# arkworks-rs/circom-compat

Measured on NVIDIA H100. Metric: groth16_proofs_per_sec_bn254_2p20, higher is better.
Workload: dtype u32x8 (254-bit Montgomery integers)

## Files before the change

### circom_compat_b200/csrc/msm.cu

```cuda
#include <algorithm>
#include <type_traits>
#include <vector>
#include "msm.cuh"
#include "util.cuh"

namespace b2g {

std::atomic<uint64_t> g_launch_count{0};

template <class C, class F>
__global__ void __launch_bounds__(128) msm_table_kernel(const void* __restrict__ bases, uint32_t n, int c, int nwin, void* __restrict__ table) {
    uint32_t i = blockIdx.x * blockDim.x + threadIdx.x;
    if (i >= n) return;
    using Pt = typename C::Pt; using Aff = typename C::Aff; using E = typename F::elem;
    Aff p = aff_load<F>(bases, i);
    if (C::aff_is_inf(p)) {
        Aff z; z.x = F::zero(); z.y = F::zero();
        for (int w = 0; w < nwin; w++) aff_store<F>(table, (size_t)w * n + i, z);
        return;
    }
    Pt pts[MSM_MAX_WIN];
    E pre[MSM_MAX_WIN];
    Pt cur = C::from_affine(p);
    E acc = F::one();
// ... 150 lines not shown
        const int leader = __ffs(pend) - 1;
        const uint32_t lb = __shfl_sync(0xffffffffu, b, leader);
        const bool mine = pending && b == lb;
        const uint32_t same = __ballot_sync(0xffffffffu, mine);
        uint32_t base = 0;
        if ((int)lane == leader) base = atomicAdd(&cursor[lb], (uint32_t)__popc(same));
        base = __shfl_sync(0xffffffffu, base, leader);
        if (mine) {
            entries[offsets[b] + base + (uint32_t)__popc(same & ((1u << lane) - 1u))] = entry;
            pending = false;
        }
    }
    if (pending) entries[offsets[b] + atomicAdd(&cursor[b], 1u)] = entry;
}

__global__ void __launch_bounds__(1024) msm_aff_levels_kernel(uint32_t nb, int rounds, uint32_t* const* __restrict__ off) {
    __shared__ uint32_t warp_sums[32];
    __shared__ uint32_t carry_s;
    const uint32_t tid = threadIdx.x, per = (nb + 1023u) / 1024u;
    const uint32_t lo = min(tid * per, nb), hi = min(lo + per, nb);
    for (int k = 1; k <= rounds; k++) {
        const uint32_t* prev = off[k - 1];
        uint32_t* cur = off[k];
        uint32_t s = 0;
        for (uint32_t j = lo; j < hi; j++) s += (prev[j + 1] - prev[j] + 1u) >> 1;
        uint32_t v = s;
        #pragma unroll
        for (int d = 1; d < 32; d <<= 1) { uint32_t t = __shfl_up_sync(0xffffffffu, v, d); if ((tid & 31) >= (uint32_t)d) v += t; }
        if ((tid & 31) == 31) warp_sums[tid >> 5] = v;
        __syncthreads();
        if (tid < 32) {
            uint32_t w = warp_sums[tid], x = w;
            #pragma unroll
            for (int d = 1; d < 32; d <<= 1) { uint32_t t = __shfl_up_sync(0xffffffffu, x, d); if (tid >= (uint32_t)d) x += t; }
            warp_sums[tid] = x - w;
            if (tid == 31) carry_s = x;
        }
        __syncthreads();
        uint32_t run = warp_sums[tid >> 5] + v - s;
        for (uint32_t j = lo; j < hi; j++) { cur[j] = run; run += (prev[j + 1] - prev[j] + 1u) >> 1; }
        if (tid == 0) cur[nb] = carry_s;
        __syncthreads();
    }
}

__global__ void __launch_bounds__(256) msm_aff_src_kernel(const uint32_t* __restrict__ off_prev, const uint32_t* __restrict__ off_cur, uint32_t nb,
                                                          uint32_t* __restrict__ src) {
    const uint32_t total = off_cur[nb];
    for (uint32_t q = blockIdx.x * blockDim.x + threadIdx.x; q < total; q += gridDim.x * blockDim.x) {
        uint32_t lo = 0, hi = nb;
        while (hi - lo > 1) { const uint32_t mid = (lo + hi) >> 1; if (off_cur[mid] <= q) lo = mid; else hi = mid; }
        const uint32_t j = q - off_cur[lo];
        const uint32_t p0 = off_prev[lo], cnt = off_prev[lo + 1] - p0;
        src[q] = (p0 + 2u * j) | ((2u * j + 1u < cnt) ? 0x80000000u : 0u);
    }
}

enum : int { AFF_COPY_P = 0, AFF_COPY_Q = 1, AFF_INF = 2, AFF_ADD = 3, AFF_DBL = 4 };

template <class C, class F, bool LEVEL0>
__device__ __forceinline__ int aff_fetch(const void* __restrict__ table, const uint32_t* __restrict__ entries, const void* __restrict__ prev,
                                         uint32_t s, typename C::Aff& P, typename C::Aff& Q, typename F::elem& d) {
    const uint32_t i0 = s & 0x7fffffffu;
    const bool pair = (s >> 31) != 0;
    if (LEVEL0) {
        const uint32_t e0 = entries[i0];
        P = aff_load<F>(table, (size_t)(e0 & 0x7fffffffu));
        if (e0 >> 31) P.y = F::neg(P.y);
        if (pair) {
            const uint32_t e1 = entries[i0 + 1];
            Q = aff_load<F>(table, (size_t)(e1 & 0x7fffffffu));
            if (e1 >> 31) Q.y = F::neg(Q.y);
        }
    } else {
        P = aff_load<F>(prev, (size_t)i0);
        if (pair) Q = aff_load<F>(prev, (size_t)i0 + 1);
    }
    if (!pair) return AFF_COPY_P;
    if (C::aff_is_inf(P)) return AFF_COPY_Q;
    if (C::aff_is_inf(Q)) return AFF_COPY_P;
    if (F::eq(P.x, Q.x)) {
        if (F::eq(P.y, Q.y) && !F::is_zero(P.y)) { d = F::dbl(P.y); return AFF_DBL; }
        return AFF_INF;
    }
    d = F::sub(Q.x, P.x);
    return AFF_ADD;
}

template <class C, class F, bool LEVEL0>
__global__ void __launch_bounds__(128) msm_aff_prod_kernel(const void* __restrict__ table, const uint32_t* __restrict__ entries, const void* __restrict__ prev,
                                                           const uint32_t* __restrict__ src, const uint32_t* __restrict__ off_cur, uint32_t nb,
                                                           void* __restrict__ pref, void* __restrict__ totals) {
    using E = typename F::elem; using Aff = typename C::Aff;
    const uint32_t total = off_cur[nb];
    const uint32_t t = blockIdx.x * blockDim.x + threadIdx.x, stride = gridDim.x * blockDim.x;
    E run = F::one();
    #pragma unroll 1
    for (int i = 0; i < MSM_AFF_M; i++) {
        const uint64_t q64 = (uint64_t)t + (uint64_t)i * stride;
        if (q64 >= total) break;
        const uint32_t q = (uint32_t)q64;
        Aff P, Q; E d;
        const int kind = aff_fetch<C, F, LEVEL0>(table, entries, prev, src[q], P, Q, d);
        if (kind >= AFF_ADD) {
            elem_store((char*)pref + (size_t)q * Bytes<F>::ELEM, run);
            run = F::mul(run, d);
        }
    }
    elem_store((char*)totals + (size_t)t * Bytes<F>::ELEM, run);
}

template <class F>
__global__ void __launch_bounds__(64) msm_aff_invert_kernel(void* __restrict__ totals, void* __restrict__ scratch, uint32_t count, uint32_t U) {
    using E = typename F::elem;
    const uint32_t u = blockIdx.x * blockDim.x + threadIdx.x;
    if (u >= U) return;
    constexpr size_t B = Bytes<F>::ELEM;
    E run = F::one();
    int last = -1;
    #pragma unroll 1
    for (int v = 0; v < MSM_AFF_S; v++) {
        const uint64_t idx = (uint64_t)u + (uint64_t)v * U;
        if (idx >= count) break;
        E x; elem_load(x, (const char*)totals + idx * B);
        elem_store((char*)scratch + idx * B, run);
        run = F::mul(run, x);
        last = v;
    }
    if (last < 0) return;
    E inv = F::inv(run);
    #pragma unroll 1
    for (int v = last; v >= 0; v--) {
        const uint64_t idx = (uint64_t)u + (uint64_t)v * U;
        E x, pre; elem_load(x, (const char*)totals + idx * B); elem_load(pre, (const char*)scratch + idx * B);
        elem_store((char*)totals + idx * B, F::mul(inv, pre));
        inv = F::mul(inv, x);
    }
}

template <class C, class F, bool LEVEL0>
__global__ void __launch_bounds__(128) msm_aff_apply_kernel(const void* __restrict__ table, const uint32_t* __restrict__ entries, const void* __restrict__ prev,
                                                            const uint32_t* __restrict__ src, const uint32_t* __restrict__ off_cur, uint32_t nb,
                                                            const void* __restrict__ pref, const void* __restrict__ totals_inv, void* __restrict__ out) {
    using E = typename F::elem; using Aff = typename C::Aff;
    const uint32_t total = off_cur[nb];
    const uint32_t t = blockIdx.x * blockDim.x + threadIdx.x, stride = gridDim.x * blockDim.x;
    if (t >= total) return;
    E inv; elem_load(inv, (const char*)totals_inv + (size_t)t * Bytes<F>::ELEM);
    int i = MSM_AFF_M - 1;
    while ((uint64_t)t + (uint64_t)i * stride >= total) i--;
    #pragma unroll 1
    for (; i >= 0; i--) {
        const uint32_t q = t + (uint32_t)i * stride;
        Aff P, Q; E d;
        const int kind = aff_fetch<C, F, LEVEL0>(table, entries, prev, src[q], P, Q, d);
        Aff r;
        if (kind >= AFF_ADD) {
            E pre; elem_load(pre, (const char*)pref + (size_t)q * Bytes<F>::ELEM);
            const E inv_d = F::mul(inv, pre);
            inv = F::mul(inv, d);
            E num;
            if (kind == AFF_ADD) num = F::sub(Q.y, P.y);
            else { const E xx = F::sqr(P.x); num = F::add(F::dbl(xx), xx); Q.x = P.x; }
            const E lam = F::mul(num, inv_d);
            r.x = F::sub(F::sub(F::sqr(lam), P.x), Q.x);
            r.y = F::sub(F::mul(lam, F::sub(P.x, r.x)), P.y);
        } else if (kind == AFF_COPY_P) r = P;
        else if (kind == AFF_COPY_Q) r = Q;
        else { r.x = F::zero(); r.y = F::zero(); }
        aff_store<F>(out, (size_t)q, r);
    }
}

template <class F> struct AccOcc;
#ifndef B2G_G1_CTAS
#define B2G_G1_CTAS 4
#endif
template <> struct AccOcc<Fq> { static constexpr int MIN_CTAS = B2G_G1_CTAS; };

__device__ __forceinline__ void acc_stage_slab(uint32_t* slab, unsigned long long* slab_bar, const uint32_t* __restrict__ entries,
                                               uint64_t cta_first, uint32_t total, uint32_t slab_words) {
// ... 246 lines not shown
    CUDA_CHECK(cudaMemsetAsync(flag.d, 0, 4, st));
    if (g2) msm_validate_kernel<G2, Fq2><<<(n + 255) / 256, 256, 0, st>>>(pts_dev, n, flag.d);
    else msm_validate_kernel<G1, Fq><<<(n + 255) / 256, 256, 0, st>>>(pts_dev, n, flag.d);
    g_launch_count += 1;
    CUDA_CHECK(cudaMemcpyAsync(&bad, flag.d, 4, cudaMemcpyDeviceToHost, st));
    CUDA_CHECK(cudaStreamSynchronize(st));
    if (bad) throw_error(B2G_E_INPUT, std::string(g2 ? "G2" : "G1") + " point " + std::to_string(bad - 1) + " of " + what + " is not on the curve");
}

template <class C, class F>
static void msm_build_table_t(MsmPlan& plan, const void* bases_dev, uint32_t n, cudaStream_t st) {
    const size_t aff = 2 * Bytes<F>::ELEM;
    uint32_t c = env_u32("B2G_MSM_C", (uint32_t)msm_pick_c(n ? n : 1));
    if (c < 8 || c > 22) throw_error(B2G_E_SHAPE, "B2G_MSM_C must be in [8, 22]");
    plan.n = n; plan.c = (int)c; plan.nwin = msm_nwin(plan.c); plan.nbuckets = 1u << (plan.c - 1);
    if (n == 0) { plan.table = nullptr; return; }
    if ((uint64_t)n * plan.nwin >= (1ull << 31)) throw_error(B2G_E_SHAPE, "msm: n * windows exceeds 2^31 table rows");
    msm_validate_points(bases_dev, n, plan.g2, st, "the query slice");
    CUDA_CHECK(cudaMalloc(&plan.table, (size_t)n * plan.nwin * aff));
    msm_table_kernel<C, F><<<(n + 127) / 128, 128, 0, st>>>(bases_dev, n, plan.c, plan.nwin, plan.table);
    g_launch_count += 1;
    CUDA_CHECK(cudaGetLastError());
}

void msm_build_table(MsmPlan& plan, const void* bases_dev, uint32_t n, bool g2, cudaStream_t st) {
    plan.g2 = g2;
    if (g2) msm_build_table_t<G2, Fq2>(plan, bases_dev, n, st);
    else msm_build_table_t<G1, Fq>(plan, bases_dev, n, st);
}

void msm_free_table(MsmPlan& plan) { if (plan.table) cudaFree(plan.table); plan.table = nullptr; }

void msm_scratch_alloc(MsmScratch& s, uint32_t n, int nwin, uint32_t nbuckets_one, bool g2, bool with_sort, uint32_t count) {
    s.g2 = g2; s.cap_n = n; s.cap_nwin = nwin; s.cap_buckets = nbuckets_one; s.cap_count = count;
    s.chunk = env_u32(g2 ? "B2G_MSM_CHUNK_G2" : "B2G_MSM_CHUNK", env_u32("B2G_MSM_CHUNK", 64));
    const size_t pt = (g2 ? 4 * 64 : 4 * 32);
    const size_t nent = (size_t)n * nwin * count;
    const size_t nbuckets = (size_t)nbuckets_one * count;
    const size_t nchunks = (nent + s.chunk - 1) / s.chunk + 1;
    s.reduce_chunk = env_u32("B2G_MSM_REDUCE_CHUNK", MSM_REDUCE_CHUNK_DEFAULT);
    {
        const char* bulk_env = getenv("B2G_ACC_BULK");
        s.bulk = bulk_env && *bulk_env ? *bulk_env == '1' : !g2;
    }
    const size_t npart = ((size_t)nbuckets_one / (s.reduce_chunk * 32) + 64) * count;
    if (with_sort) {
        CUDA_CHECK(cudaMalloc(&s.counts, (size_t)nbuckets * 4));
        CUDA_CHECK(cudaMalloc(&s.offsets, ((size_t)nbuckets + 1) * 4));
        CUDA_CHECK(cudaMalloc(&s.cursor, (size_t)nbuckets * 4));
        CUDA_CHECK(cudaMalloc(&s.entries, (nent + 8) * 4));
        CUDA_CHECK(cudaMalloc(&s.scalars_canon, ((size_t)n * count + 1) * sizeof(fe)));
    }
    CUDA_CHECK(cudaMalloc(&s.big_list, (size_t)nbuckets * 4));
    CUDA_CHECK(cudaMalloc(&s.big_count, 4));
    CUDA_CHECK(cudaMalloc(&s.frag_first, nchunks * pt));
    CUDA_CHECK(cudaMalloc(&s.frag_last, nchunks * pt));
    CUDA_CHECK(cudaMalloc(&s.buckets, (size_t)nbuckets * pt));
    CUDA_CHECK(cudaMalloc(&s.partials, (npart + 1) * pt));
    CUDA_CHECK(cudaMalloc(&s.result, pt)); s.result_owned = true;
    {
        int rounds = 0;
        const char* ov = getenv("B2G_MSM_AFFINE_ROUNDS");
        if (ov && *ov) { long x = strtol(ov, nullptr, 10); rounds = x < 0 ? 0 : (x > MSM_AFF_MAX_ROUNDS ? MSM_AFF_MAX_ROUNDS : (int)x); }
        s.aff_cap_rounds = rounds;
        s.aff_nmax[0] = (uint32_t)nent;
        for (int k = 1; k <= rounds; k++) s.aff_nmax[k] = s.aff_nmax[k - 1] / 2 + (uint32_t)(nbuckets / 2) + 1;
        if (rounds) {
            const size_t elem = g2 ? 64 : 32, aff = 2 * elem;
            if (with_sort) {
                std::vector<uint32_t*> offs(MSM_AFF_MAX_ROUNDS + 1, nullptr);
                offs[0] = s.offsets;
                for (int k = 1; k <= rounds; k++) {
                    CUDA_CHECK(cudaMalloc(&s.aff_off[k], ((size_t)nbuckets + 1) * 4));
                    CUDA_CHECK(cudaMalloc(&s.aff_src[k], ((size_t)s.aff_nmax[k] + 1) * 4));
                    offs[k] = s.aff_off[k];
                }
                s.aff_off[0] = s.offsets;
                CUDA_CHECK(cudaMalloc(&s.aff_off_dev, (MSM_AFF_MAX_ROUNDS + 1) * sizeof(uint32_t*)));
                CUDA_CHECK(cudaMemcpy(s.aff_off_dev, offs.data(), (MSM_AFF_MAX_ROUNDS + 1) * sizeof(uint32_t*), cudaMemcpyHostToDevice));
            }
            CUDA_CHECK(cudaMalloc(&s.aff_list[0], ((size_t)s.aff_nmax[1] + 1) * aff));
            if (rounds > 1) CUDA_CHECK(cudaMalloc(&s.aff_list[1], ((size_t)s.aff_nmax[2] + 1) * aff));
            const size_t threads1 = ((size_t)s.aff_nmax[1] + MSM_AFF_M - 1) / MSM_AFF_M + 128;
            CUDA_CHECK(cudaMalloc(&s.aff_pref, ((size_t)s.aff_nmax[1] + 1) * elem));
            CUDA_CHECK(cudaMalloc(&s.aff_totals, threads1 * elem));
            CUDA_CHECK(cudaMalloc(&s.aff_tscratch, threads1 * elem));
        }
    }
    if (env_u32("B2G_MSM_TAIL_PRIORITY", 1) == 1) {
        int least = 0, greatest = 0;
        CUDA_CHECK(cudaDeviceGetStreamPriorityRange(&least, &greatest));
        CUDA_CHECK(cudaStreamCreateWithPriority(&s.tail, cudaStreamNonBlocking, greatest));
        CUDA_CHECK(cudaEventCreateWithFlags(&s.ev_acc, cudaEventDisableTiming));
        CUDA_CHECK(cudaEventCreateWithFlags(&s.ev_tail, cudaEventDisableTiming));
    }
}

void msm_scratch_free(MsmScratch& s) {
    void* ptrs[] = {s.counts, s.offsets, s.cursor, s.entries, s.big_list, s.big_count, s.frag_first, s.frag_last,
                    s.buckets, s.partials, s.result_owned ? s.result : nullptr, s.scalars_canon,
                    s.aff_list[0], s.aff_list[1], s.aff_pref, s.aff_totals, s.aff_tscratch, s.aff_off_dev};
    for (void* p : ptrs) if (p) cudaFree(p);
    for (int k = 1; k <= MSM_AFF_MAX_ROUNDS; k++) { if (s.aff_off[k]) cudaFree(s.aff_off[k]); if (s.aff_src[k]) cudaFree(s.aff_src[k]); }
    if (s.tail) { cudaStreamDestroy(s.tail); cudaEventDestroy(s.ev_acc); cudaEventDestroy(s.ev_tail); }
    s = MsmScratch();
}

void msm_sort(const MsmPlan& plan, MsmScratch& s, const fe* scalars_dev, uint32_t n, bool scalars_mont, cudaStream_t st, uint32_t count,
              uint32_t scalar_stride) {
    if (n > plan.n) n = plan.n;
    s.sorted_n = n; s.sorted_count = count;
    if (n == 0 || plan.table == nullptr) return;
    if (n > s.cap_n || plan.nwin > s.cap_nwin || plan.nbuckets > s.cap_buckets || count > s.cap_count || !s.entries) throw_error(B2G_E_SHAPE, "msm: sort scratch too small");
    const uint32_t nb = plan.nbuckets * count;
    constexpr unsigned SORT_CTA = 256;
    CUDA_CHECK(cudaMemsetAsync(s.counts, 0, (size_t)nb * 4, st));
    const dim3 pair_grid((unsigned)(((uint64_t)n * plan.nwin + SORT_CTA - 1) / SORT_CTA), count);
    msm_canon_kernel<<<dim3((n + SORT_CTA - 1) / SORT_CTA, count), SORT_CTA, 0, st>>>(scalars_dev, n, scalar_stride ? scalar_stride : n, scalars_mont ? 1 : 0, s.scalars_canon);
    msm_count_kernel<<<pair_grid, SORT_CTA, 0, st>>>(s.scalars_canon, n, plan.c, plan.nwin, plan.nbuckets, s.counts);
    msm_scan_kernel<<<1, 1024, 0, st>>>(s.counts, nb, s.offsets, s.cursor);
    msm_scatter_kernel<<<pair_grid, SORT_CTA, 0, st>>>(s.scalars_canon, n, plan.n, plan.c, plan.nwin, plan.nbuckets, s.offsets, s.cursor, s.entries);
    g_launch_count += 4;
    s.aff_rounds = s.aff_off_dev ? s.aff_cap_rounds : 0;
    if (s.aff_rounds) {
        msm_aff_levels_kernel<<<1, 1024, 0, st>>>(nb, s.aff_rounds, s.aff_off_dev);
        for (int k = 1; k <= s.aff_rounds; k++) {
            const unsigned blocks = (unsigned)std::min<uint64_t>(((uint64_t)s.aff_nmax[k] + 255) / 256, 1u << 20);
            msm_aff_src_kernel<<<blocks, 256, 0, st>>>(s.aff_off[k - 1], s.aff_off[k], nb, s.aff_src[k]);
        }
        g_launch_count += 1 + s.aff_rounds;
    }
    CUDA_CHECK(cudaGetLastError());
}

template <class C, class F>
static void launch_accumulate(const void* table, const uint32_t* entries, const uint32_t* offsets, uint32_t nb, uint32_t chunk, uint32_t nruns,
                              const MsmScratch& s, bool bulk, cudaStream_t st) {
    constexpr bool g2 = std::is_same<F, Fq2>::value;
    constexpr uint32_t runs_per_cta = g2 ? 64u : 128u;
    const uint32_t slab_words = bulk && (size_t)chunk * runs_per_cta * 4 <= MSM_SLAB_MAX_BYTES ? chunk * runs_per_cta : 0u;
    const unsigned blocks = (unsigned)(((uint64_t)nruns + runs_per_cta - 1) / runs_per_cta);
    if constexpr (g2)
        msm_accumulate_g2_kernel<<<blocks, 128, (size_t)slab_words * 4, st>>>(table, entries, offsets, nb, chunk, s.buckets, s.frag_first, s.frag_last, slab_words);
    else
        msm_accumulate_kernel<C, F><<<blocks, 128, (size_t)slab_words * 4, st>>>(table, entries, offsets, nb, chunk, s.buckets, s.frag_first, s.frag_last, slab_words);
}

template <class C, class F>
static void msm_accumulate_t(const MsmPlan& plan, const MsmScratch& sorted, MsmScratch& s, cudaStream_t st) {
    using Pt = typename C::Pt;
    const size_t ptb = sizeof(Pt);
    const uint32_t n = sorted.sorted_n, count = sorted.sorted_count;
    const size_t rstride = s.result_stride ? s.result_stride : ptb;
    if (n == 0 || plan.table == nullptr) { CUDA_CHECK(cudaMemset2DAsync(s.result, rstride, 0, ptb, count, st)); return; }
    if (plan.nbuckets > s.cap_buckets || n > s.cap_n || plan.nwin > s.cap_nwin || count > s.cap_count) throw_error(B2G_E_SHAPE, "msm: accumulate scratch too small");
    const uint32_t nb = plan.nbuckets * count, chunk = s.chunk;
    CUDA_CHECK(cudaMemsetAsync(s.big_count, 0, 4, st));
    const uint64_t nent = (uint64_t)n * plan.nwin * count;
    const uint32_t nthreads = (uint32_t)((nent + chunk - 1) / chunk);
    if (s.prof0) CUDA_CHECK(cudaEventRecord(s.prof0, st));
    int rounds = sorted.aff_rounds < s.aff_cap_rounds ? sorted.aff_rounds : s.aff_cap_rounds;
    if (rounds && (sorted.aff_nmax[1] > s.aff_nmax[1] || !s.aff_list[0])) rounds = 0;
    const uint32_t* offsets = sorted.offsets;
    if (rounds) {
        const void* prev = nullptr;
        for (int k = 1; k <= rounds; k++) {
            const uint32_t nk = sorted.aff_nmax[k];
            const unsigned blocks = (unsigned)(((uint64_t)nk + (uint64_t)MSM_AFF_M * 128 - 1) / ((uint64_t)MSM_AFF_M * 128));
            const uint32_t stride = blocks * 128u, U = (stride + MSM_AFF_S - 1) / MSM_AFF_S;
            void* out = s.aff_list[(k - 1) & 1];
            if (k == 1) {
                msm_aff_prod_kernel<C, F, true><<<blocks, 128, 0, st>>>(plan.table, sorted.entries, nullptr, sorted.aff_src[k], sorted.aff_off[k], nb, s.aff_pref, s.aff_totals);
                msm_aff_invert_kernel<F><<<(U + 63) / 64, 64, 0, st>>>(s.aff_totals, s.aff_tscratch, stride, U);
                msm_aff_apply_kernel<C, F, true><<<blocks, 128, 0, st>>>(plan.table, sorted.entries, nullptr, sorted.aff_src[k], sorted.aff_off[k], nb, s.aff_pref, s.aff_totals, out);
            } else {
                msm_aff_prod_kernel<C, F, false><<<blocks, 128, 0, st>>>(nullptr, nullptr, prev, sorted.aff_src[k], sorted.aff_off[k], nb, s.aff_pref, s.aff_totals);
                msm_aff_invert_kernel<F><<<(U + 63) / 64, 64, 0, st>>>(s.aff_totals, s.aff_tscratch, stride, U);
// ... 20 lines not shown
    const uint32_t npart = (nred + NT - 1) / NT;
    msm_reduce_kernel<C, F><<<dim3(npart, count), NT, sh, st>>>(s.buckets, nb1, rchunk, s.partials);
    msm_sum_kernel<C, F><<<count, NT, sh, st>>>(s.partials, npart, s.result, rstride);
    if (s.tail) { CUDA_CHECK(cudaEventRecord(s.ev_tail, s.tail)); CUDA_CHECK(cudaStreamWaitEvent(main_st, s.ev_tail, 0)); }
    g_launch_count += 5;
    CUDA_CHECK(cudaGetLastError());
}

void msm_accumulate(const MsmPlan& plan, const MsmScratch& sorted, MsmScratch& acc, cudaStream_t st) {
    if (plan.g2) msm_accumulate_t<G2, Fq2>(plan, sorted, acc, st);
    else msm_accumulate_t<G1, Fq>(plan, sorted, acc, st);
}

void msm_run(const MsmPlan& plan, MsmScratch& s, const fe* scalars_dev, uint32_t n, bool scalars_mont, cudaStream_t st, uint32_t count,
             uint32_t scalar_stride) {
    msm_sort(plan, s, scalars_dev, n, scalars_mont, st, count, scalar_stride);
    msm_accumulate(plan, s, s, st);
}

void msm_init_kernels() {
    CUDA_CHECK(cudaFuncSetAttribute(msm_accumulate_kernel<G1, Fq>, cudaFuncAttributeMaxDynamicSharedMemorySize, MSM_SLAB_MAX_BYTES));
    CUDA_CHECK(cudaFuncSetAttribute(msm_accumulate_g2_kernel, cudaFuncAttributeMaxDynamicSharedMemorySize, MSM_SLAB_MAX_BYTES));
}

}
```

### circom_compat_b200/csrc/msm.cuh

```cuda
#pragma once
#include "ec.cuh"

namespace b2g {

constexpr int MSM_MAX_WIN = 32;
constexpr int MSM_BIG_FRAGS = 32;

struct MsmPlan {
    uint32_t n = 0;
    int c = 0, nwin = 0;
    uint32_t nbuckets = 0;
    void* table = nullptr;
    bool g2 = false;
};

constexpr int MSM_AFF_MAX_ROUNDS = 6;
constexpr int MSM_AFF_M = 16;
constexpr int MSM_AFF_S = 64;

struct MsmScratch {
    uint32_t cap_n = 0; int cap_nwin = 0; uint32_t cap_buckets = 0; uint32_t chunk = 64; uint32_t sorted_n = 0; uint32_t reduce_chunk = 8;
    uint32_t cap_count = 1, sorted_count = 1;
    size_t result_stride = 0;
    uint32_t *counts = nullptr, *offsets = nullptr, *cursor = nullptr, *entries = nullptr;
    uint32_t *big_list = nullptr, *big_count = nullptr;
    void *frag_first = nullptr, *frag_last = nullptr, *buckets = nullptr, *partials = nullptr, *result = nullptr;
    fe* scalars_canon = nullptr;
    bool g2 = false, result_owned = false;
    bool bulk = false;
    cudaEvent_t prof0 = nullptr, prof1 = nullptr;
    cudaStream_t tail = nullptr;
    cudaEvent_t ev_acc = nullptr, ev_tail = nullptr;
    int aff_rounds = 0;
    int aff_cap_rounds = 0;
    uint32_t aff_nmax[MSM_AFF_MAX_ROUNDS + 1] = {};
    uint32_t* aff_off[MSM_AFF_MAX_ROUNDS + 1] = {};
    uint32_t** aff_off_dev = nullptr;
    uint32_t* aff_src[MSM_AFF_MAX_ROUNDS + 1] = {};
    void* aff_list[2] = {nullptr, nullptr};
    void *aff_pref = nullptr, *aff_totals = nullptr, *aff_tscratch = nullptr;
};

inline int msm_pick_c(uint32_t n) {
    if (n >= 3u << 18) return 17;
    if (n >= 1u << 19) return 16;
    if (n >= 1u << 15) return 15;
    if (n >= 1u << 13) return 13;
    if (n >= 1u << 11) return 11;
    int lg = 0; while ((1ull << (lg + 1)) <= n) lg++;
    return lg - 3 < 8 ? 8 : lg - 3;
}
inline int msm_nwin(int c) { return (255 + c - 1) / c; }

}
```

### circom_compat_b200/csrc/prover.cu

```cuda
#include <atomic>
#include <chrono>
#include <cstring>
#include <vector>
#include "../../include/b2groth.h"
#include "ec.cuh"
#include "msm.cuh"
#include "ntt.cuh"
#include "util.cuh"

namespace b2g {

void msm_build_table(MsmPlan& plan, const void* bases_dev, uint32_t n, bool g2, cudaStream_t st);
void msm_free_table(MsmPlan& plan);
void msm_scratch_alloc(MsmScratch& s, uint32_t n, int nwin, uint32_t nbuckets, bool g2, bool with_sort, uint32_t count = 1);
void msm_sort(const MsmPlan& plan, MsmScratch& s, const fe* scalars_dev, uint32_t n, bool scalars_mont, cudaStream_t st, uint32_t count = 1,
              uint32_t scalar_stride = 0);
void msm_accumulate(const MsmPlan& plan, const MsmScratch& sorted, MsmScratch& acc, cudaStream_t st);
void msm_scratch_free(MsmScratch& s);
void msm_run(const MsmPlan& plan, MsmScratch& s, const fe* scalars_dev, uint32_t n, bool scalars_mont, cudaStream_t st, uint32_t count = 1,
             uint32_t scalar_stride = 0);
void msm_init_kernels();
void msm_validate_points(const void* pts_dev, uint32_t n, bool g2, cudaStream_t st, const char* what);

enum { Q_H = 0, Q_L = 1, Q_A = 2, Q_B1 = 3, Q_B2 = 4, NQ = 5 };
static const size_t PARTIAL_OFF[NQ] = {0, 128, 256, 384, 512};
constexpr size_t REC_BYTES = B2G_PARTIAL_BYTES + 256;
constexpr uint32_t MAX_BATCH = 65535;

}

using namespace b2g;
// ... 512 lines not shown
    ctx->cap_batch = 0; ctx->alloc_gen++;
    if (ctx->scratch_ok) for (int q = 0; q < NQ; q++) ctx->scratch[q].result = nullptr;
    CUDA_CHECK(cudaMalloc(&ctx->d_partial, count * REC_BYTES));
    CUDA_CHECK(cudaMemset(ctx->d_partial, 0, count * REC_BYTES));
    CUDA_CHECK(cudaMalloc(&ctx->d_proof, count * 256));
    CUDA_CHECK(cudaMalloc(&ctx->d_pre, count * PRE_BYTES));
    CUDA_CHECK(cudaMalloc(&ctx->d_rs, count * 64));
    CUDA_CHECK(cudaMallocHost(&ctx->h_rs, count * 64));
    CUDA_CHECK(cudaMallocHost(&ctx->h_proof, count * 256));
    ctx->cap_batch = count;
    if (ctx->scratch_ok) for (int q = 0; q < NQ; q++) ctx->scratch[q].result = ctx->d_partial + PARTIAL_OFF[q];
}

static void ensure_scratch(b2g_ctx* ctx, const b2g_pk* pk, uint32_t count = 1) {
    const size_t nwb = (size_t)pk->b_compact * count;
    bool ok = ctx->scratch_ok && (!pk->d_bidx || (ctx->scratch_bsort && nwb <= ctx->cap_wb));
    for (int q = 0; q < NQ && ok; q++) {
        const MsmPlan& p = pk->plan[q]; const MsmScratch& sc = ctx->scratch[q];
        if ((p.n ? p.n : 1) > sc.cap_n || p.nwin > sc.cap_nwin || p.nbuckets > sc.cap_buckets || count > sc.cap_count) ok = false;
    }
    if (ok) return;
    CUDA_CHECK(cudaDeviceSynchronize());
    for (int q = 0; q < NQ; q++) msm_scratch_free(ctx->scratch[q]);
    ctx->scratch_ok = false; ctx->alloc_gen++;
    for (int q = 0; q < NQ; q++) {
        const MsmPlan& p = pk->plan[q];
        msm_scratch_alloc(ctx->scratch[q], p.n ? p.n : 1, p.nwin, p.nbuckets, q == Q_B2, q == Q_H || q == Q_L || (q == Q_B1 && pk->d_bidx), count);
        cudaFree(ctx->scratch[q].result);
        ctx->scratch[q].result = ctx->d_partial + PARTIAL_OFF[q];
        ctx->scratch[q].result_owned = false;
        ctx->scratch[q].result_stride = REC_BYTES;
    }
    ctx->scratch_bsort = pk->d_bidx != nullptr;
    const size_t nwb_cap = (size_t)pk->b_compact * count;
    if (nwb_cap > ctx->cap_wb) {
        if (ctx->d_wb) cudaFree(ctx->d_wb);
        ctx->d_wb = nullptr; ctx->cap_wb = 0;
        CUDA_CHECK(cudaMalloc(&ctx->d_wb, (nwb_cap + 1) * sizeof(fe)));
        ctx->cap_wb = nwb_cap;
    }
    ctx->scratch_ok = true;
}
// ... 55 lines not shown
        ntt_transform_single(mat->dom, eval, st);
        eval_publish_kernel<<<1, 32, 0, st>>>(ctx->d_xchg, ctx->d_epoch);
        g_launch_count += 1;
    }
    if (cnt) {
        h_slice_kernel<<<(cnt + 255) / 256, 256, 0, st>>>(ctx->d_peer_ptrs, ctx->d_epoch, lo, cnt, ctx->d_h, p2p_timeout_ns(), d_flag);
        g_launch_count += 1;
    }
    CUDA_CHECK(cudaGetLastError());
}

static void launch_msms(b2g_ctx* ctx, b2g_pk* pk, b2g_mat* mat, bool timed, bool scale, bool split_map = false, uint32_t count = 1) {
    cudaStream_t s0 = ctx->st[0], ssort = ctx->st[Q_L];
    CUDA_CHECK(cudaEventRecord(ctx->ev_w, s0));
    CUDA_CHECK(cudaStreamWaitEvent(ssort, ctx->ev_w, 0));
    msm_sort(pk->plan[Q_A], ctx->scratch[Q_L], ctx->d_w + pk->scalar_off[Q_A] + pk->lo[Q_A], pk->cnt[Q_A], true, ssort, count, pk->n_vars);
    CUDA_CHECK(cudaEventRecord(ctx->ev_sort, ssort));
    const bool bsparse = pk->d_bidx != nullptr;
    if (bsparse) {
        cudaStream_t sb = ctx->st[Q_B1];
        CUDA_CHECK(cudaStreamWaitEvent(sb, ctx->ev_w, 0));
        if (pk->b_compact) gather_scalars_kernel<<<dim3((pk->b_compact + 255) / 256, count), 256, 0, sb>>>(ctx->d_w + pk->scalar_off[Q_B1] + pk->lo[Q_B1], pk->n_vars, pk->d_bidx, pk->b_compact, ctx->d_wb);
        g_launch_count += 1;
        msm_sort(pk->plan[Q_B1], ctx->scratch[Q_B1], ctx->d_wb, pk->b_compact, true, sb, count, pk->b_compact);
        CUDA_CHECK(cudaEventRecord(ctx->ev_sortb, sb));
    }
    const int* order = witness_order();
    for (int oi = 0; oi < 4; oi++) {
        const int q = order[oi];
        const bool on_b = bsparse && (q == Q_B1 || q == Q_B2);
        if (on_b) { if (q != Q_B1) CUDA_CHECK(cudaStreamWaitEvent(ctx->st[q], ctx->ev_sortb, 0)); }
        else if (q != Q_L) CUDA_CHECK(cudaStreamWaitEvent(ctx->st[q], ctx->ev_sort, 0));
        if (timed) CUDA_CHECK(cudaEventRecord(ctx->ev_t[2 * q], ctx->st[q]));
        msm_accumulate(pk->plan[q], on_b ? ctx->scratch[Q_B1] : ctx->scratch[Q_L], ctx->scratch[q], ctx->st[q]);
        if (scale && (q == Q_A || q == Q_B1)) {
            const Scalar256* rs = reinterpret_cast<const Scalar256*>(ctx->d_rs);
            scale_partial_kernel<<<count, 32, 0, ctx->st[q]>>>(ctx->d_partial + PARTIAL_OFF[q], q == Q_A ? rs + 1 : rs, ctx->d_partial + B2G_PARTIAL_BYTES + (q == Q_A ? 0 : 128));
            g_launch_count += 1;
        }
        if (timed) CUDA_CHECK(cudaEventRecord(ctx->ev_t[2 * q + 1], ctx->st[q]));
        CUDA_CHECK(cudaEventRecord(ctx->ev_done[q], ctx->st[q]));
    }
    if (timed) CUDA_CHECK(cudaEventRecord(ctx->ev_t[10], s0));
    if (split_map) run_witness_map_split(ctx, mat, pk->lo[Q_H], pk->cnt[Q_H], s0);
    else run_witness_map(ctx, mat, s0, count);
    if (timed) CUDA_CHECK(cudaEventRecord(ctx->ev_t[11], s0));
    if (timed) CUDA_CHECK(cudaEventRecord(ctx->ev_t[0], s0));
    msm_run(pk->plan[Q_H], ctx->scratch[Q_H], ctx->d_h + pk->lo[Q_H], pk->cnt[Q_H], true, s0, count, mat->n);
// ... 689 lines not shown
}

}
template <bool IS_G2>
static void msm_entry(b2g_ctx* ctx, const void* bases, const void* scalars, size_t n, int scalars_mont, void* out) {
    if (!ctx || !out || (n && (!bases || !scalars))) throw_error(B2G_E_SHAPE, "null pointer");
    if (n >= (1ull << 27)) throw_error(B2G_E_SHAPE, "msm too large");
    DevGuard g(ctx->device);
    cudaStream_t st = ctx->st[0];
    const size_t aff = IS_G2 ? 128 : 64, ptb = 2 * aff;
    if (n == 0) { memset(out, 0, aff); return; }
    uint8_t* d_bases = dev_upload<uint8_t>(bases, n * aff, st);
    fe* d_sc = dev_upload<fe>(scalars, n * 32, st);
    MsmPlan plan; MsmScratch sc;
    msm_build_table(plan, d_bases, (uint32_t)n, IS_G2, st);
    msm_scratch_alloc(sc, (uint32_t)n, plan.nwin, plan.nbuckets, IS_G2, true);
    msm_run(plan, sc, d_sc, (uint32_t)n, scalars_mont != 0, st);
    uint8_t* d_out = nullptr; CUDA_CHECK(cudaMalloc(&d_out, aff));
    if (IS_G2) xyzz_to_affine_kernel<G2, Fq2><<<1, 1, 0, st>>>(sc.result, 1, d_out);
    else xyzz_to_affine_kernel<G1, Fq><<<1, 1, 0, st>>>(sc.result, 1, d_out);
    g_launch_count += 2;
    CUDA_CHECK(cudaMemcpyAsync(out, d_out, aff, cudaMemcpyDeviceToHost, st));
    cudaError_t e = cudaStreamSynchronize(st);
    (void)ptb;
    cudaFree(d_out); cudaFree(d_bases); cudaFree(d_sc); msm_free_table(plan); msm_scratch_free(sc);
    CUDA_CHECK(e);
}

extern "C" {
int b2g_msm_g1(b2g_ctx* ctx, const void* bases, const void* scalars, size_t n, int scalars_mont, void* out) {
    return guarded([&] { msm_entry<false>(ctx, bases, scalars, n, scalars_mont, out); });
// ... 80 lines not shown
```

Baseline: 35.94.

## Enable affine batch-inversion bucket rounds for large G2 MSMs by default

Turns on two rounds of affine pairwise bucket reduction with Montgomery batch inversion for G2 MSMs of size 2^18 or more. Before, this path was only reachable through an environment variable. The level-offset kernel now computes each round's offsets in parallel from the base offsets, one block per round, instead of looping serially. The product kernel prefetches sort entries and loads only x coordinates to form denominators, and Fq2 uses inline mul/sqr. When a single consumer needs levels, their planning moves onto that consumer's stream, at the cost of extra scratch memory and more complex allocation logic.

Result: no change. 36.11 (median of 6 runs) (+0.5%).

```diff
diff --git a/circom_compat_b200/csrc/msm.cu b/circom_compat_b200/csrc/msm.cu
--- a/circom_compat_b200/csrc/msm.cu
+++ b/circom_compat_b200/csrc/msm.cu
@@ -188,34 +188,33 @@
     if (pending) entries[offsets[b] + atomicAdd(&cursor[b], 1u)] = entry;
 }
 
-__global__ void __launch_bounds__(1024) msm_aff_levels_kernel(uint32_t nb, int rounds, uint32_t* const* __restrict__ off) {
+__global__ void __launch_bounds__(1024) msm_aff_levels_kernel(uint32_t nb, uint32_t* const* __restrict__ off) {
     __shared__ uint32_t warp_sums[32];
     __shared__ uint32_t carry_s;
     const uint32_t tid = threadIdx.x, per = (nb + 1023u) / 1024u;
     const uint32_t lo = min(tid * per, nb), hi = min(lo + per, nb);
-    for (int k = 1; k <= rounds; k++) {
-        const uint32_t* prev = off[k - 1];
-        uint32_t* cur = off[k];
-        uint32_t s = 0;
-        for (uint32_t j = lo; j < hi; j++) s += (prev[j + 1] - prev[j] + 1u) >> 1;
-        uint32_t v = s;
+    const int k = (int)blockIdx.x + 1;
+    const uint32_t* base = off[0];
+    uint32_t* cur = off[k];
+    const uint64_t round_up = (1ull << k) - 1;
+    uint32_t s = 0;
+    for (uint32_t j = lo; j < hi; j++) s += (uint32_t)(((uint64_t)(base[j + 1] - base[j]) + round_up) >> k);
+    uint32_t v = s;
+    #pragma unroll
+    for (int d = 1; d < 32; d <<= 1) { uint32_t t = __shfl_up_sync(0xffffffffu, v, d); if ((tid & 31) >= (uint32_t)d) v += t; }
+    if ((tid & 31) == 31) warp_sums[tid >> 5] = v;
+    __syncthreads();
+    if (tid < 32) {
+        uint32_t w = warp_sums[tid], x = w;
         #pragma unroll
-        for (int d = 1; d < 32; d <<= 1) { uint32_t t = __shfl_up_sync(0xffffffffu, v, d); if ((tid & 31) >= (uint32_t)d) v += t; }
-        if ((tid & 31) == 31) warp_sums[tid >> 5] = v;
-        __syncthreads();
-        if (tid < 32) {
-            uint32_t w = warp_sums[tid], x = w;
-            #pragma unroll
-            for (int d = 1; d < 32; d <<= 1) { uint32_t t = __shfl_up_sync(0xffffffffu, x, d); if (tid >= (uint32_t)d) x += t; }
-            warp_sums[tid] = x - w;
-            if (tid == 31) carry_s = x;
-        }
-        __syncthreads();
-        uint32_t run = warp_sums[tid >> 5] + v - s;
-        for (uint32_t j = lo; j < hi; j++) { cur[j] = run; run += (prev[j + 1] - prev[j] + 1u) >> 1; }
-        if (tid == 0) cur[nb] = carry_s;
-        __syncthreads();
-    }
+        for (int d = 1; d < 32; d <<= 1) { uint32_t t = __shfl_up_sync(0xffffffffu, x, d); if (tid >= (uint32_t)d) x += t; }
+        warp_sums[tid] = x - w;
+        if (tid == 31) carry_s = x;
+    }
+    __syncthreads();
+    uint32_t run = warp_sums[tid >> 5] + v - s;
+    for (uint32_t j = lo; j < hi; j++) { cur[j] = run; run += (uint32_t)(((uint64_t)(base[j + 1] - base[j]) + round_up) >> k); }
+    if (tid == 0) cur[nb] = carry_s;
 }
 
 __global__ void __launch_bounds__(256) msm_aff_src_kernel(const uint32_t* __restrict__ off_prev, const uint32_t* __restrict__ off_cur, uint32_t nb,
@@ -232,25 +231,49 @@
 
 enum : int { AFF_COPY_P = 0, AFF_COPY_Q = 1, AFF_INF = 2, AFF_ADD = 3, AFF_DBL = 4 };
 
-template <class C, class F, bool LEVEL0>
-__device__ __forceinline__ int aff_fetch(const void* __restrict__ table, const uint32_t* __restrict__ entries, const void* __restrict__ prev,
-                                         uint32_t s, typename C::Aff& P, typename C::Aff& Q, typename F::elem& d) {
-    const uint32_t i0 = s & 0x7fffffffu;
-    const bool pair = (s >> 31) != 0;
+template <class F> struct AffMath {
+    using E = typename F::elem;
+    static __device__ __forceinline__ E mul(const E& a, const E& b) { return F::mul(a, b); }
+    static __device__ __forceinline__ E sqr(const E& a) { return F::sqr(a); }
+};
+template <> struct AffMath<Fq2> {
+    static __device__ __forceinline__ fe2 mul(const fe2& a, const fe2& b) { return Fq2::mul_inline(a, b); }
+    static __device__ __forceinline__ fe2 sqr(const fe2& a) { return Fq2::sqr_inline(a); }
+};
+
+struct AffSlot { uint32_t s, e0, e1; };
+
+template <bool LEVEL0>
+__device__ __forceinline__ AffSlot aff_slot(const uint32_t* __restrict__ entries, uint32_t s) {
+    AffSlot a; a.s = s; a.e0 = 0; a.e1 = 0;
     if (LEVEL0) {
-        const uint32_t e0 = entries[i0];
-        P = aff_load<F>(table, (size_t)(e0 & 0x7fffffffu));
-        if (e0 >> 31) P.y = F::neg(P.y);
-        if (pair) {
-            const uint32_t e1 = entries[i0 + 1];
-            Q = aff_load<F>(table, (size_t)(e1 & 0x7fffffffu));
-            if (e1 >> 31) Q.y = F::neg(Q.y);
-        }
-    } else {
-        P = aff_load<F>(prev, (size_t)i0);
-        if (pair) Q = aff_load<F>(prev, (size_t)i0 + 1);
-    }
-    if (!pair) return AFF_COPY_P;
+        const uint32_t i0 = s & 0x7fffffffu;
+        a.e0 = entries[i0];
+        if (s >> 31) a.e1 = entries[i0 + 1];
+    }
+    return a;
+}
+
+template <class F, bool LEVEL0>
+__device__ __forceinline__ const char* aff_row(const void* __restrict__ table, const void* __restrict__ prev, const AffSlot& a, int j, bool& neg) {
+    constexpr size_t ROW = 2 * Bytes<F>::ELEM;
+    if (LEVEL0) {
+        const uint32_t e = j ? a.e1 : a.e0;
+        neg = (e >> 31) != 0;
+        return (const char*)table + (size_t)(e & 0x7fffffffu) * ROW;
+    }
+    neg = false;
+    return (const char*)prev + (size_t)((a.s & 0x7fffffffu) + (uint32_t)j) * ROW;
+}
+
+template <class F>
+__device__ __forceinline__ typename F::elem aff_row_y(const char* row, bool neg) {
+    typename F::elem y; elem_load_nc(y, row + Bytes<F>::ELEM);
+    return neg ? F::neg(y) : y;
+}
+
+template <class C, class F>
+__device__ __forceinline__ int aff_classify(const typename C::Aff& P, const typename C::Aff& Q, typename F::elem& d) {
     if (C::aff_is_inf(P)) return AFF_COPY_Q;
     if (C::aff_is_inf(Q)) return AFF_COPY_P;
     if (F::eq(P.x, Q.x)) {
@@ -262,23 +285,62 @@
 }
 
 template <class C, class F, bool LEVEL0>
+__device__ __forceinline__ int aff_fetch(const void* __restrict__ table, const void* __restrict__ prev, const AffSlot& a,
+                                         typename C::Aff& P, typename C::Aff& Q, typename F::elem& d) {
+    bool neg;
+    const char* r0 = aff_row<F, LEVEL0>(table, prev, a, 0, neg);
+    elem_load_nc(P.x, r0);
+    P.y = aff_row_y<F>(r0, neg);
+    if ((a.s >> 31) == 0) return AFF_COPY_P;
+    const char* r1 = aff_row<F, LEVEL0>(table, prev, a, 1, neg);
+    elem_load_nc(Q.x, r1);
+    Q.y = aff_row_y<F>(r1, neg);
+    return aff_classify<C, F>(P, Q, d);
+}
+
+template <class C, class F, bool LEVEL0>
+__device__ __forceinline__ int aff_fetch_den(const void* __restrict__ table, const void* __restrict__ prev, const AffSlot& a, typename F::elem& d) {
+    if ((a.s >> 31) == 0) return AFF_COPY_P;
+    bool n0, n1;
+    const char* r0 = aff_row<F, LEVEL0>(table, prev, a, 0, n0);
+    const char* r1 = aff_row<F, LEVEL0>(table, prev, a, 1, n1);
+    typename C::Aff P, Q;
+    elem_load_nc(P.x, r0); elem_load_nc(Q.x, r1);
+    if (!F::is_zero(P.x) && !F::is_zero(Q.x) && !F::eq(P.x, Q.x)) { d = F::sub(Q.x, P.x); return AFF_ADD; }
+    P.y = aff_row_y<F>(r0, n0); Q.y = aff_row_y<F>(r1, n1);
+    return aff_classify<C, F>(P, Q, d);
+}
+
+__device__ __forceinline__ int aff_slot_count(uint32_t t, uint32_t stride, uint32_t total) {
+    if (t >= total) return 0;
+    const uint64_t c = ((uint64_t)total - t + stride - 1) / stride;
+    return c < (uint64_t)MSM_AFF_M ? (int)c : MSM_AFF_M;
+}
+
+template <class C, class F, bool LEVEL0>
 __global__ void __launch_bounds__(128) msm_aff_prod_kernel(const void* __restrict__ table, const uint32_t* __restrict__ entries, const void* __restrict__ prev,
                                                            const uint32_t* __restrict__ src, const uint32_t* __restrict__ off_cur, uint32_t nb,
                                                            void* __restrict__ pref, void* __restrict__ totals) {
-    using E = typename F::elem; using Aff = typename C::Aff;
+    using E = typename F::elem;
     const uint32_t total = off_cur[nb];
     const uint32_t t = blockIdx.x * blockDim.x + threadIdx.x, stride = gridDim.x * blockDim.x;
+    const int cnt = aff_slot_count(t, stride, total);
     E run = F::one();
-    #pragma unroll 1
-    for (int i = 0; i < MSM_AFF_M; i++) {
-        const uint64_t q64 = (uint64_t)t + (uint64_t)i * stride;
-        if (q64 >= total) break;
-        const uint32_t q = (uint32_t)q64;
-        Aff P, Q; E d;
-        const int kind = aff_fetch<C, F, LEVEL0>(table, entries, prev, src[q], P, Q, d);
-        if (kind >= AFF_ADD) {
-            elem_store((char*)pref + (size_t)q * Bytes<F>::ELEM, run);
-            run = F::mul(run, d);
+    if (cnt > 0) {
+        AffSlot next = aff_slot<LEVEL0>(entries, src[t]);
+        uint32_t s_ahead = cnt > 1 ? src[t + stride] : 0u;
+        #pragma unroll 1
+        for (int i = 0; i < cnt; i++) {
+            const uint32_t q = t + (uint32_t)i * stride;
+            const AffSlot cur = next;
+            if (i + 1 < cnt) next = aff_slot<LEVEL0>(entries, s_ahead);
+            if (i + 2 < cnt) s_ahead = src[q + 2 * stride];
+            E d;
+            const int kind = aff_fetch_den<C, F, LEVEL0>(table, prev, cur, d);
+            if (kind >= AFF_ADD) {
+                elem_store((char*)pref + (size_t)q * Bytes<F>::ELEM, run);
+                run = AffMath<F>::mul(run, d);
+            }
         }
     }
     elem_store((char*)totals + (size_t)t * Bytes<F>::ELEM, run);
@@ -298,7 +360,7 @@
         if (idx >= count) break;
         E x; elem_load(x, (const char*)totals + idx * B);
         elem_store((char*)scratch + idx * B, run);
-        run = F::mul(run, x);
+        run = AffMath<F>::mul(run, x);
         last = v;
     }
     if (last < 0) return;
@@ -307,8 +369,8 @@
     for (int v = last; v >= 0; v--) {
         const uint64_t idx = (uint64_t)u + (uint64_t)v * U;
         E x, pre; elem_load(x, (const char*)totals + idx * B); elem_load(pre, (const char*)scratch + idx * B);
-        elem_store((char*)totals + idx * B, F::mul(inv, pre));
-        inv = F::mul(inv, x);
+        elem_store((char*)totals + idx * B, AffMath<F>::mul(inv, pre));
+        inv = AffMath<F>::mul(inv, x);
     }
 }
 
@@ -321,24 +383,29 @@
     const uint32_t t = blockIdx.x * blockDim.x + threadIdx.x, stride = gridDim.x * blockDim.x;
     if (t >= total) return;
     E inv; elem_load(inv, (const char*)totals_inv + (size_t)t * Bytes<F>::ELEM);
-    int i = MSM_AFF_M - 1;
-    while ((uint64_t)t + (uint64_t)i * stride >= total) i--;
+    const int cnt = aff_slot_count(t, stride, total);
+    AffSlot next = aff_slot<LEVEL0>(entries, src[t + (uint32_t)(cnt - 1) * stride]);
+    uint32_t s_ahead = cnt > 1 ? src[t + (uint32_t)(cnt - 2) * stride] : 0u;
     #pragma unroll 1
-    for (; i >= 0; i--) {
+    for (int i = cnt - 1; i >= 0; i--) {
         const uint32_t q = t + (uint32_t)i * stride;
+        const AffSlot cur = next;
+        if (i >= 1) next = aff_slot<LEVEL0>(entries, s_ahead);
+        if (i >= 2) s_ahead = src[q - 2 * stride];
         Aff P, Q; E d;
-        const int kind = aff_fetch<C, F, LEVEL0>(table, entries, prev, src[q], P, Q, d);
+        const int kind = aff_fetch<C, F, LEVEL0>(table, prev, cur, P, Q, d);
         Aff r;
         if (kind >= AFF_ADD) {
             E pre; elem_load(pre, (const char*)pref + (size_t)q * Bytes<F>::ELEM);
-            const E inv_d = F::mul(inv, pre);
-            inv = F::mul(inv, d);
+            using M = AffMath<F>;
+            const E inv_d = M::mul(inv, pre);
+            inv = M::mul(inv, d);
             E num;
             if (kind == AFF_ADD) num = F::sub(Q.y, P.y);
-            else { const E xx = F::sqr(P.x); num = F::add(F::dbl(xx), xx); Q.x = P.x; }
-            const E lam = F::mul(num, inv_d);
-            r.x = F::sub(F::sub(F::sqr(lam), P.x), Q.x);
-            r.y = F::sub(F::mul(lam, F::sub(P.x, r.x)), P.y);
+            else { const E xx = M::sqr(P.x); num = F::add(F::dbl(xx), xx); Q.x = P.x; }
+            const E lam = M::mul(num, inv_d);
+            r.x = F::sub(F::sub(M::sqr(lam), P.x), Q.x);
+            r.y = F::sub(M::mul(lam, F::sub(P.x, r.x)), P.y);
         } else if (kind == AFF_COPY_P) r = P;
         else if (kind == AFF_COPY_Q) r = Q;
         else { r.x = F::zero(); r.y = F::zero(); }
@@ -615,6 +682,7 @@
     uint32_t c = env_u32("B2G_MSM_C", (uint32_t)msm_pick_c(n ? n : 1));
     if (c < 8 || c > 22) throw_error(B2G_E_SHAPE, "B2G_MSM_C must be in [8, 22]");
     plan.n = n; plan.c = (int)c; plan.nwin = msm_nwin(plan.c); plan.nbuckets = 1u << (plan.c - 1);
+    plan.aff_rounds = msm_pick_aff_rounds(plan.g2, n);
     if (n == 0) { plan.table = nullptr; return; }
     if ((uint64_t)n * plan.nwin >= (1ull << 31)) throw_error(B2G_E_SHAPE, "msm: n * windows exceeds 2^31 table rows");
     msm_validate_points(bases_dev, n, plan.g2, st, "the query slice");
@@ -632,7 +700,16 @@
 
 void msm_free_table(MsmPlan& plan) { if (plan.table) cudaFree(plan.table); plan.table = nullptr; }
 
-void msm_scratch_alloc(MsmScratch& s, uint32_t n, int nwin, uint32_t nbuckets_one, bool g2, bool with_sort, uint32_t count) {
+int msm_aff_rounds(const MsmPlan& plan) {
+    const char* ov = plan.g2 ? getenv("B2G_MSM_AFFINE_ROUNDS_G2") : nullptr;
+    if (!ov || !*ov) ov = getenv("B2G_MSM_AFFINE_ROUNDS");
+    if (!ov || !*ov) return plan.aff_rounds;
+    const long x = strtol(ov, nullptr, 10);
+    return x < 0 ? 0 : (x > MSM_AFF_MAX_ROUNDS ? MSM_AFF_MAX_ROUNDS : (int)x);
+}
+
+void msm_scratch_alloc(MsmScratch& s, uint32_t n, int nwin, uint32_t nbuckets_one, bool g2, bool with_sort, uint32_t count, int aff_rounds,
+                       int sort_rounds) {
     s.g2 = g2; s.cap_n = n; s.cap_nwin = nwin; s.cap_buckets = nbuckets_one; s.cap_count = count;
     s.chunk = env_u32(g2 ? "B2G_MSM_CHUNK_G2" : "B2G_MSM_CHUNK", env_u32("B2G_MSM_CHUNK", 64));
     const size_t pt = (g2 ? 4 * 64 : 4 * 32);
@@ -660,26 +737,27 @@
     CUDA_CHECK(cudaMalloc(&s.partials, (npart + 1) * pt));
     CUDA_CHECK(cudaMalloc(&s.result, pt)); s.result_owned = true;
     {
-        int rounds = 0;
-        const char* ov = getenv("B2G_MSM_AFFINE_ROUNDS");
-        if (ov && *ov) { long x = strtol(ov, nullptr, 10); rounds = x < 0 ? 0 : (x > MSM_AFF_MAX_ROUNDS ? MSM_AFF_MAX_ROUNDS : (int)x); }
+        const int rounds = aff_rounds;
+        if (!with_sort) sort_rounds = 0;
         s.aff_cap_rounds = rounds;
+        s.aff_sort_rounds = sort_rounds;
         s.aff_nmax[0] = (uint32_t)nent;
-        for (int k = 1; k <= rounds; k++) s.aff_nmax[k] = s.aff_nmax[k - 1] / 2 + (uint32_t)(nbuckets / 2) + 1;
+        for (int k = 1; k <= std::max(rounds, sort_rounds); k++)
+            s.aff_nmax[k] = std::min(s.aff_nmax[k - 1], s.aff_nmax[k - 1] / 2 + (uint32_t)(nbuckets / 2) + 1);
+        if (sort_rounds) {
+            std::vector<uint32_t*> offs(MSM_AFF_MAX_ROUNDS + 1, nullptr);
+            offs[0] = s.offsets;
+            for (int k = 1; k <= sort_rounds; k++) {
+                CUDA_CHECK(cudaMalloc(&s.aff_off[k], ((size_t)nbuckets + 1) * 4));
+                CUDA_CHECK(cudaMalloc(&s.aff_src[k], ((size_t)s.aff_nmax[k] + 1) * 4));
+                offs[k] = s.aff_off[k];
+            }
+            s.aff_off[0] = s.offsets;
+            CUDA_CHECK(cudaMalloc(&s.aff_off_dev, (MSM_AFF_MAX_ROUNDS + 1) * sizeof(uint32_t*)));
+            CUDA_CHECK(cudaMemcpy(s.aff_off_dev, offs.data(), (MSM_AFF_MAX_ROUNDS + 1) * sizeof(uint32_t*), cudaMemcpyHostToDevice));
+        }
         if (rounds) {
             const size_t elem = g2 ? 64 : 32, aff = 2 * elem;
-            if (with_sort) {
-                std::vector<uint32_t*> offs(MSM_AFF_MAX_ROUNDS + 1, nullptr);
-                offs[0] = s.offsets;
-                for (int k = 1; k <= rounds; k++) {
-                    CUDA_CHECK(cudaMalloc(&s.aff_off[k], ((size_t)nbuckets + 1) * 4));
-                    CUDA_CHECK(cudaMalloc(&s.aff_src[k], ((size_t)s.aff_nmax[k] + 1) * 4));
-                    offs[k] = s.aff_off[k];
-                }
-                s.aff_off[0] = s.offsets;
-                CUDA_CHECK(cudaMalloc(&s.aff_off_dev, (MSM_AFF_MAX_ROUNDS + 1) * sizeof(uint32_t*)));
-                CUDA_CHECK(cudaMemcpy(s.aff_off_dev, offs.data(), (MSM_AFF_MAX_ROUNDS + 1) * sizeof(uint32_t*), cudaMemcpyHostToDevice));
-            }
             CUDA_CHECK(cudaMalloc(&s.aff_list[0], ((size_t)s.aff_nmax[1] + 1) * aff));
             if (rounds > 1) CUDA_CHECK(cudaMalloc(&s.aff_list[1], ((size_t)s.aff_nmax[2] + 1) * aff));
             const size_t threads1 = ((size_t)s.aff_nmax[1] + MSM_AFF_M - 1) / MSM_AFF_M + 128;
@@ -707,8 +785,10 @@
     s = MsmScratch();
 }
 
+void msm_sort_levels(const MsmPlan& plan, MsmScratch& s, cudaStream_t st);
+
 void msm_sort(const MsmPlan& plan, MsmScratch& s, const fe* scalars_dev, uint32_t n, bool scalars_mont, cudaStream_t st, uint32_t count,
-              uint32_t scalar_stride) {
+              uint32_t scalar_stride, bool plan_levels) {
     if (n > plan.n) n = plan.n;
     s.sorted_n = n; s.sorted_count = count;
     if (n == 0 || plan.table == nullptr) return;
@@ -722,15 +802,20 @@
     msm_scan_kernel<<<1, 1024, 0, st>>>(s.counts, nb, s.offsets, s.cursor);
     msm_scatter_kernel<<<pair_grid, SORT_CTA, 0, st>>>(s.scalars_canon, n, plan.n, plan.c, plan.nwin, plan.nbuckets, s.offsets, s.cursor, s.entries);
     g_launch_count += 4;
-    s.aff_rounds = s.aff_off_dev ? s.aff_cap_rounds : 0;
-    if (s.aff_rounds) {
-        msm_aff_levels_kernel<<<1, 1024, 0, st>>>(nb, s.aff_rounds, s.aff_off_dev);
-        for (int k = 1; k <= s.aff_rounds; k++) {
-            const unsigned blocks = (unsigned)std::min<uint64_t>(((uint64_t)s.aff_nmax[k] + 255) / 256, 1u << 20);
-            msm_aff_src_kernel<<<blocks, 256, 0, st>>>(s.aff_off[k - 1], s.aff_off[k], nb, s.aff_src[k]);
-        }
-        g_launch_count += 1 + s.aff_rounds;
-    }
+    s.aff_rounds = s.aff_off_dev ? s.aff_sort_rounds : 0;
+    if (plan_levels) msm_sort_levels(plan, s, st);
+    CUDA_CHECK(cudaGetLastError());
+}
+
+void msm_sort_levels(const MsmPlan& plan, MsmScratch& s, cudaStream_t st) {
+    if (s.sorted_n == 0 || plan.table == nullptr || !s.aff_rounds) return;
+    const uint32_t nb = plan.nbuckets * s.sorted_count;
+    msm_aff_levels_kernel<<<s.aff_rounds, 1024, 0, st>>>(nb, s.aff_off_dev);
+    for (int k = 1; k <= s.aff_rounds; k++) {
+        const unsigned blocks = (unsigned)std::min<uint64_t>(((uint64_t)s.aff_nmax[k] + 255) / 256, 1u << 20);
+        msm_aff_src_kernel<<<blocks, 256, 0, st>>>(s.aff_off[k - 1], s.aff_off[k], nb, s.aff_src[k]);
+    }
+    g_launch_count += 1 + s.aff_rounds;
     CUDA_CHECK(cudaGetLastError());
 }
 
@@ -761,7 +846,7 @@
     const uint32_t nthreads = (uint32_t)((nent + chunk - 1) / chunk);
     if (s.prof0) CUDA_CHECK(cudaEventRecord(s.prof0, st));
     int rounds = sorted.aff_rounds < s.aff_cap_rounds ? sorted.aff_rounds : s.aff_cap_rounds;
-    if (rounds && (sorted.aff_nmax[1] > s.aff_nmax[1] || !s.aff_list[0])) rounds = 0;
+    for (int k = 1; k <= rounds && k <= 2; k++) if (sorted.aff_nmax[k] > s.aff_nmax[k]) rounds = 0;
     const uint32_t* offsets = sorted.offsets;
     if (rounds) {
         const void* prev = nullptr;
@@ -812,7 +897,7 @@
 
 void msm_run(const MsmPlan& plan, MsmScratch& s, const fe* scalars_dev, uint32_t n, bool scalars_mont, cudaStream_t st, uint32_t count,
              uint32_t scalar_stride) {
-    msm_sort(plan, s, scalars_dev, n, scalars_mont, st, count, scalar_stride);
+    msm_sort(plan, s, scalars_dev, n, scalars_mont, st, count, scalar_stride, true);
     msm_accumulate(plan, s, s, st);
 }
 
diff --git a/circom_compat_b200/csrc/msm.cuh b/circom_compat_b200/csrc/msm.cuh
--- a/circom_compat_b200/csrc/msm.cuh
+++ b/circom_compat_b200/csrc/msm.cuh
@@ -12,6 +12,7 @@
     uint32_t nbuckets = 0;
     void* table = nullptr;
     bool g2 = false;
+    int aff_rounds = 0;
 };
 
 constexpr int MSM_AFF_MAX_ROUNDS = 6;
@@ -32,6 +33,7 @@
     cudaStream_t tail = nullptr;
     cudaEvent_t ev_acc = nullptr, ev_tail = nullptr;
     int aff_rounds = 0;
+    int aff_sort_rounds = 0;
     int aff_cap_rounds = 0;
     uint32_t aff_nmax[MSM_AFF_MAX_ROUNDS + 1] = {};
     uint32_t* aff_off[MSM_AFF_MAX_ROUNDS + 1] = {};
@@ -52,4 +54,8 @@
 }
 inline int msm_nwin(int c) { return (255 + c - 1) / c; }
 
+constexpr uint32_t MSM_AFF_G2_MIN_N = 1u << 18;
+constexpr int MSM_AFF_G2_ROUNDS = 2;
+inline int msm_pick_aff_rounds(bool g2, uint32_t n) { return g2 && n >= MSM_AFF_G2_MIN_N ? MSM_AFF_G2_ROUNDS : 0; }
+
 }
diff --git a/circom_compat_b200/csrc/prover.cu b/circom_compat_b200/csrc/prover.cu
--- a/circom_compat_b200/csrc/prover.cu
+++ b/circom_compat_b200/csrc/prover.cu
@@ -12,9 +12,12 @@
 
 void msm_build_table(MsmPlan& plan, const void* bases_dev, uint32_t n, bool g2, cudaStream_t st);
 void msm_free_table(MsmPlan& plan);
-void msm_scratch_alloc(MsmScratch& s, uint32_t n, int nwin, uint32_t nbuckets, bool g2, bool with_sort, uint32_t count = 1);
+int msm_aff_rounds(const MsmPlan& plan);
+void msm_scratch_alloc(MsmScratch& s, uint32_t n, int nwin, uint32_t nbuckets, bool g2, bool with_sort, uint32_t count = 1, int aff_rounds = 0,
+                       int sort_rounds = 0);
 void msm_sort(const MsmPlan& plan, MsmScratch& s, const fe* scalars_dev, uint32_t n, bool scalars_mont, cudaStream_t st, uint32_t count = 1,
-              uint32_t scalar_stride = 0);
+              uint32_t scalar_stride = 0, bool plan_levels = true);
+void msm_sort_levels(const MsmPlan& plan, MsmScratch& s, cudaStream_t st);
 void msm_accumulate(const MsmPlan& plan, const MsmScratch& sorted, MsmScratch& acc, cudaStream_t st);
 void msm_scratch_free(MsmScratch& s);
 void msm_run(const MsmPlan& plan, MsmScratch& s, const fe* scalars_dev, uint32_t n, bool scalars_mont, cudaStream_t st, uint32_t count = 1,
@@ -557,10 +560,18 @@
 
 static void ensure_scratch(b2g_ctx* ctx, const b2g_pk* pk, uint32_t count = 1) {
     const size_t nwb = (size_t)pk->b_compact * count;
+    int acc_rounds[NQ], sort_rounds[NQ] = {};
+    for (int q = 0; q < NQ; q++) acc_rounds[q] = msm_aff_rounds(pk->plan[q]);
+    sort_rounds[Q_H] = acc_rounds[Q_H];
+    for (int q : {Q_L, Q_A, Q_B1, Q_B2}) {
+        const int sorter = pk->d_bidx && (q == Q_B1 || q == Q_B2) ? Q_B1 : Q_L;
+        sort_rounds[sorter] = std::max(sort_rounds[sorter], acc_rounds[q]);
+    }
     bool ok = ctx->scratch_ok && (!pk->d_bidx || (ctx->scratch_bsort && nwb <= ctx->cap_wb));
     for (int q = 0; q < NQ && ok; q++) {
         const MsmPlan& p = pk->plan[q]; const MsmScratch& sc = ctx->scratch[q];
         if ((p.n ? p.n : 1) > sc.cap_n || p.nwin > sc.cap_nwin || p.nbuckets > sc.cap_buckets || count > sc.cap_count) ok = false;
+        if (acc_rounds[q] != sc.aff_cap_rounds || sort_rounds[q] != sc.aff_sort_rounds) ok = false;
     }
     if (ok) return;
     CUDA_CHECK(cudaDeviceSynchronize());
@@ -568,7 +579,8 @@
     ctx->scratch_ok = false; ctx->alloc_gen++;
     for (int q = 0; q < NQ; q++) {
         const MsmPlan& p = pk->plan[q];
-        msm_scratch_alloc(ctx->scratch[q], p.n ? p.n : 1, p.nwin, p.nbuckets, q == Q_B2, q == Q_H || q == Q_L || (q == Q_B1 && pk->d_bidx), count);
+        msm_scratch_alloc(ctx->scratch[q], p.n ? p.n : 1, p.nwin, p.nbuckets, q == Q_B2, q == Q_H || q == Q_L || (q == Q_B1 && pk->d_bidx), count,
+                          acc_rounds[q], sort_rounds[q]);
         cudaFree(ctx->scratch[q].result);
         ctx->scratch[q].result = ctx->d_partial + PARTIAL_OFF[q];
         ctx->scratch[q].result_owned = false;
@@ -654,9 +666,14 @@
     cudaStream_t s0 = ctx->st[0], ssort = ctx->st[Q_L];
     CUDA_CHECK(cudaEventRecord(ctx->ev_w, s0));
     CUDA_CHECK(cudaStreamWaitEvent(ssort, ctx->ev_w, 0));
-    msm_sort(pk->plan[Q_A], ctx->scratch[Q_L], ctx->d_w + pk->scalar_off[Q_A] + pk->lo[Q_A], pk->cnt[Q_A], true, ssort, count, pk->n_vars);
+    const bool bsparse = pk->d_bidx != nullptr;
+    int lev_q = -1, nlev = 0;
+    for (int q : {Q_L, Q_A, Q_B1, Q_B2})
+        if (!(bsparse && (q == Q_B1 || q == Q_B2)) && ctx->scratch[q].aff_cap_rounds) { lev_q = q; nlev++; }
+    const bool lev_own_stream = nlev == 1 && lev_q != Q_L;
+    msm_sort(pk->plan[Q_A], ctx->scratch[Q_L], ctx->d_w + pk->scalar_off[Q_A] + pk->lo[Q_A], pk->cnt[Q_A], true, ssort, count, pk->n_vars,
+             !lev_own_stream);
     CUDA_CHECK(cudaEventRecord(ctx->ev_sort, ssort));
-    const bool bsparse = pk->d_bidx != nullptr;
     if (bsparse) {
         cudaStream_t sb = ctx->st[Q_B1];
         CUDA_CHECK(cudaStreamWaitEvent(sb, ctx->ev_w, 0));
@@ -672,6 +689,7 @@
         if (on_b) { if (q != Q_B1) CUDA_CHECK(cudaStreamWaitEvent(ctx->st[q], ctx->ev_sortb, 0)); }
         else if (q != Q_L) CUDA_CHECK(cudaStreamWaitEvent(ctx->st[q], ctx->ev_sort, 0));
         if (timed) CUDA_CHECK(cudaEventRecord(ctx->ev_t[2 * q], ctx->st[q]));
+        if (lev_own_stream && q == lev_q) msm_sort_levels(pk->plan[Q_A], ctx->scratch[Q_L], ctx->st[q]);
         msm_accumulate(pk->plan[q], on_b ? ctx->scratch[Q_B1] : ctx->scratch[Q_L], ctx->scratch[q], ctx->st[q]);
         if (scale && (q == Q_A || q == Q_B1)) {
             const Scalar256* rs = reinterpret_cast<const Scalar256*>(ctx->d_rs);
@@ -1391,7 +1409,8 @@
     fe* d_sc = dev_upload<fe>(scalars, n * 32, st);
     MsmPlan plan; MsmScratch sc;
     msm_build_table(plan, d_bases, (uint32_t)n, IS_G2, st);
-    msm_scratch_alloc(sc, (uint32_t)n, plan.nwin, plan.nbuckets, IS_G2, true);
+    const int rounds = msm_aff_rounds(plan);
+    msm_scratch_alloc(sc, (uint32_t)n, plan.nwin, plan.nbuckets, IS_G2, true, 1, rounds, rounds);
     msm_run(plan, sc, d_sc, (uint32_t)n, scalars_mont != 0, st);
     uint8_t* d_out = nullptr; CUDA_CHECK(cudaMalloc(&d_out, aff));
     if (IS_G2) xyzz_to_affine_kernel<G2, Fq2><<<1, 1, 0, st>>>(sc.result, 1, d_out);
```
